# NVIDIA-ISAAC-ROS/isaac_ros_nvblox

Measured on NVIDIA H100. Metric: depth-frames/sec (TSDF+ESDF integrate, 640x480 @ 5 cm voxels), higher is better.
Workload: dtype f32

## Files before the change

### isaac_ros_nvblox_b200/csrc/nvb_esdf_wavex.cu

```cuda
#include "nvb_esdf_wave_common.cuh"

#include <cstdlib>

namespace nvb {

namespace {

#ifndef NVB_WAVEX_THREADS
#define NVB_WAVEX_THREADS 512
#endif
#ifndef NVB_WAVEX_MAXREG
#define NVB_WAVEX_MAXREG 96
#endif
#ifndef NVB_WAVEX_TAIL
#define NVB_WAVEX_TAIL 1
#endif
#ifndef NVB_WAVEX_PROF
#define NVB_WAVEX_PROF 0
#endif
#ifndef NVB_WAVEX_SPEC_HALO
#define NVB_WAVEX_SPEC_HALO 0
#endif
#if NVB_WAVEX_PROF
#define X_PROF_BEGIN() long long tq = clock64();
#define X_PROF(i) \
  if (lane64 == 0) xs.prof[group][i] += clock64() - tq; \
  tq = clock64();
#define X_PROF_COUNT(i) \
  if (lane64 == 0) xs.prof[group][i]++;
#else
#define X_PROF_BEGIN()
#define X_PROF(i)
#define X_PROF_COUNT(i)
#endif
constexpr int kXT = NVB_WAVEX_THREADS;
constexpr int kXG = kXT / 64;
constexpr int kRecInts = 32;
constexpr int kMaxCtas = 192;
constexpr int kRX = 110, kRY = 11;
constexpr int kRegionVox = 1100;
constexpr int kFlagBase = 4 * kRegionVox;
constexpr int kXRegionWords = 5 * kRegionVox;
constexpr size_t kXSmemBytes = (size_t)kXG * kXRegionWords * sizeof(unsigned int);

struct XTables {
  unsigned int halo[8][64];
  unsigned int pair[6][4][64];
};

struct XShared {
  int rec[kXG][kRecInts];
  int nb[kXG][8];
  int pos[kXG][8];
  unsigned int mask[kXG];
  int changed[kXG];
  unsigned int live[kXG][8];
  int seg[kXG][2];
  int pre[kMaxCtas + 1];
  int warp_tot[2][8];
  int ncand, nchanged;
  int next;
  int cur[kXG];
  int seeds[kXG];
  int bcast[4];
  unsigned int generation;
  int n_bar;
  int ring;
  int swept, faces, rings, n_tail;
#if NVB_WAVEX_PROF
  long long prof[kXG][8];
#endif
};

struct XCtx {
  unsigned char* blocks;
  int* block_index;
  DevHash hash;
  int* nbr;
  int* nbr27;
  int* cand_stamp;
  unsigned int* psum;
  int* stamp[2];
  unsigned char* X[2];
  int* recs[2];
  int seg;
  int* error;
  float max_sq;
  __device__ __forceinline__ int* segment(int p, int cta) const { return recs[p] + (size_t)cta * seg * kRecInts; }
};

__shared__ XTables x_tab;
__shared__ XShared x_xs;
__shared__ XCtx x_ctx;
extern __shared__ __align__(16) unsigned int x_smem[];

__device__ __forceinline__ int rvox(int rx, int ry, int rz) { return rx * kRX + ry * kRY + rz; }
__device__ __forceinline__ int faceEntry(int f) {
  return f == 0 ? 22 : (f == 1 ? 4 : (f == 2 ? 16 : (f == 3 ? 10 : (f == 4 ? 14 : 12))));
}
__device__ __forceinline__ int boundaryOff(int r) { return r == 0 ? -1 : (r == 9 ? 1 : 0); }
__device__ __forceinline__ int boundaryLoc(int r) { return r == 0 ? 7 : (r == 9 ? 0 : r - 1); }

__device__ __forceinline__ int neighbor27(const XCtx& c, int slot, int d) {
  int v = __ldcg(c.nbr27 + 27 * slot + d);
  if (v < -1) {
    const int* bi = c.block_index + 3 * slot;
    v = (d == 13) ? slot : hashFind(c.hash, bi[0] + d / 9 - 1, bi[1] + (d / 3) % 3 - 1, bi[2] + d % 3 - 1);
    c.nbr27[27 * slot + d] = v;
  }
  return v;
}
__device__ __forceinline__ int neighbor6(const XCtx& c, int slot, int dir) {
  int v = __ldcg(c.nbr + 6 * slot + dir);
  if (v < -1) {
    const int* bi = c.block_index + 3 * slot;
    const int d = (dir & 1) ? -1 : 1;
    v = hashFind(c.hash, bi[0] + ((dir >> 1) == 0 ? d : 0), bi[1] + ((dir >> 1) == 1 ? d : 0), bi[2] + ((dir >> 1) == 2 ? d : 0));
    c.nbr[6 * slot + dir] = v;
  }
  return v;
}

__device__ __forceinline__ void initTables(XTables& tab, int tid) {
  for (int i = tid; i < 512; i += kXT) {
    const int k = i >> 6, lane = i & 63;
    unsigned int e = 0;
    int ra = 1, r1 = 1, r2 = 1, axis = 0;
    bool valid = true;
    if (k < 6) {
      axis = k >> 1;
      ra = (k & 1) ? 0 : 9, r1 = (lane >> 3) + 1, r2 = (lane & 7) + 1;
    } else {
      const int n = i - 384;
      if (n < 96) {
        const int edge = n >> 3, cn = edge & 3;
        axis = edge >> 2;
        ra = (n & 7) + 1, r1 = (cn & 1) ? 9 : 0, r2 = (cn & 2) ? 9 : 0;
      } else if (n < 104) {
        const int cn = n - 96;
        ra = (cn & 1) ? 9 : 0, r1 = (cn & 2) ? 9 : 0, r2 = (cn & 4) ? 9 : 0;
      } else {
        valid = false;
      }
    }
    if (valid) {
      const int rx = axis == 0 ? ra : r1, ry = axis == 0 ? r1 : (axis == 1 ? ra : r2), rz = axis == 2 ? ra : r2;
      const int d = (boundaryOff(rx) + 1) * 9 + (boundaryOff(ry) + 1) * 3 + (boundaryOff(rz) + 1);
      e = (unsigned)rvox(rx, ry, rz) | ((unsigned)(boundaryLoc(rx) * 64 + boundaryLoc(ry) * 8 + boundaryLoc(rz)) << 11) |
          ((unsigned)d << 20) | (1u << 25);
    }
    tab.halo[k][lane] = e;
  }
  for (int i = tid; i < 6 * 4 * 64; i += kXT) {
    const int pass = i >> 8, j = (i >> 6) & 3, lane = i & 63;
    const int axis = pass >> 1, dir = (pass & 1) ? -1 : 1;
    int plane, u, w;
    bool valid = true;
    if (j < 2) {
      plane = j, u = (lane >> 3) + 1, w = (lane & 7) + 1;
    } else {
      const int n = (j - 2) * 64 + lane;
      plane = n / 36;
      const int q = n % 36;
      if (q < 10) u = 0, w = q;
      else if (q < 20) u = 9, w = q - 10;
      else if (q < 28) u = q - 20 + 1, w = 0;
      else u = q - 28 + 1, w = 9;
      if (n >= 72) valid = false, plane = 0, u = 1, w = 1;
    }
    unsigned int e = 0;
    if (valid) {
      const int sa = dir > 0 ? (plane ? 8 : 0) : (plane ? 9 : 1);
      const int so = dir > 0 ? (plane ? 0 : -1) : (plane ? 1 : 0);
      const int da = sa + dir;
      const int A = axis == 0 ? 9 : (axis == 1 ? 3 : 1), U = axis == 0 ? 3 : 9, W = axis == 2 ? 3 : 1;
      const int d = 13 + so * A + boundaryOff(u) * U + boundaryOff(w) * W;
      const int inner = da >= 1 && da <= 8 && u >= 1 && u <= 8 && w >= 1 && w <= 8;
      const int sv = axis == 0 ? rvox(sa, u, w) : (axis == 1 ? rvox(u, sa, w) : rvox(u, w, sa));
      const int dv = axis == 0 ? rvox(da, u, w) : (axis == 1 ? rvox(u, da, w) : rvox(u, w, da));
      e = (unsigned)sv | ((unsigned)dv << 11) | ((unsigned)d << 22) | ((unsigned)inner << 27) | (1u << 28);
    }
    tab.pair[pass][j][lane] = e;
  }
}

struct LiveMasks {
  unsigned int* live;
  unsigned int needed;
};
__device__ __forceinline__ LiveMasks liveMasks(unsigned int mask, unsigned int* live_smem, bool writer) {
  LiveMasks L;
  L.live = live_smem;
  const unsigned int ok = mask | (1u << 13);
  const unsigned int D[6] = {0x7FFFE00u, 0x3FE00u, 0x3F000u, 0x7000u, 0x6000u, 0x2000u};
  unsigned int acc = 0;
#pragma unroll
  for (int p = 0; p < 6; p++) {
    const int axis = p >> 1;
    const int A = axis == 0 ? 9 : (axis == 1 ? 3 : 1);
    const unsigned int lo = axis == 0 ? 0x000001ffu : (axis == 1 ? 0x001c0e07u : 0x01249249u);
    const unsigned int dst_ok = ok & D[p];
    unsigned int lv, dst;
    if ((p & 1) == 0) {
      lv = mask & (lo | (lo << A)) & (dst_ok >> A);
      dst = lv << A;
    } else {
      lv = mask & ((lo << A) | (lo << (2 * A))) & (dst_ok << A);
      dst = lv >> A;
    }
    if (writer) live_smem[p] = lv;
    acc |= lv | dst;
  }
  L.needed = acc & mask & ~(1u << 13);
  return L;
}

struct OwnRegs {
  uint4 q[10];
};
__device__ __forceinline__ OwnRegs ownLoad(const unsigned char* blk, int lane64) {
  OwnRegs o;
  const uint4* src = reinterpret_cast<const uint4*>(blk) + lane64 * 10;
#pragma unroll
  for (int i = 0; i < 10; i++) o.q[i] = __ldcg(src + i);
  return o;
}
__device__ __forceinline__ unsigned int ownWord(const OwnRegs& o, int w) {
  const uint4& v = o.q[w >> 2];
  return (w & 3) == 0 ? v.x : ((w & 3) == 1 ? v.y : ((w & 3) == 2 ? v.z : v.w));
}
__device__ __forceinline__ void ownToShared(unsigned int* R, const OwnRegs& o, int lane64) {
  uint4* A = reinterpret_cast<uint4*>(R);
  const int v0 = rvox((lane64 >> 3) + 1, (lane64 & 7) + 1, 1);
#pragma unroll
  for (int z = 0; z < 8; z++) {
    A[v0 + z] = make_uint4(ownWord(o, 5 * z), ownWord(o, 5 * z + 1), ownWord(o, 5 * z + 2), ownWord(o, 5 * z + 3));
    R[kFlagBase + v0 + z] = ownWord(o, 5 * z + 4);
  }
}
__device__ __forceinline__ void ownStore(unsigned char* layer_blk, bool to_layer, unsigned char* x_blk, const unsigned int* R,
                                         unsigned int* psum_slot, int lane64) {
  const uint4* A = reinterpret_cast<const uint4*>(R);
  const int x = lane64 >> 3, y = lane64 & 7;
  const int v0 = rvox(x + 1, y + 1, 1);
  uint4* dl = reinterpret_cast<uint4*>(layer_blk) + lane64 * 10;
  uint4* dx = reinterpret_cast<uint4*>(x_blk) + lane64 * 10;
  int lo0 = 99, lo1 = 99, lo2 = 99, hi0 = -99, hi1 = -99, hi2 = -99;
#pragma unroll
  for (int h = 0; h < 2; h++) {
    unsigned int w[20];
#pragma unroll
    for (int z = 0; z < 4; z++) {
      const uint4 a = A[v0 + 4 * h + z];
      w[5 * z] = a.x, w[5 * z + 1] = a.y, w[5 * z + 2] = a.z, w[5 * z + 3] = a.w;
      w[5 * z + 4] = R[kFlagBase + v0 + 4 * h + z];
      if ((a.y | a.z | a.w) != 0u) {
        const int b0 = (x + (int)a.y) >> 3, b1 = (y + (int)a.z) >> 3, b2 = (4 * h + z + (int)a.w) >> 3;
        lo0 = min(lo0, b0), hi0 = max(hi0, b0), lo1 = min(lo1, b1), hi1 = max(hi1, b1), lo2 = min(lo2, b2), hi2 = max(hi2, b2);
      }
    }
#pragma unroll
    for (int i = 0; i < 5; i++) {
      const uint4 v = make_uint4(w[4 * i], w[4 * i + 1], w[4 * i + 2], w[4 * i + 3]);
      if (to_layer) __stcg(dl + 5 * h + i, v);
      __stcg(dx + 5 * h + i, v);
    }
  }
  if (psum_slot) {
    lo0 = __reduce_min_sync(0xffffffffu, lo0), lo1 = __reduce_min_sync(0xffffffffu, lo1), lo2 = __reduce_min_sync(0xffffffffu, lo2);
    hi0 = __reduce_max_sync(0xffffffffu, hi0), hi1 = __reduce_max_sync(0xffffffffu, hi1), hi2 = __reduce_max_sync(0xffffffffu, hi2);
    if ((lane64 & 31) == 0) {
      unsigned int v = 0u;
      if (lo0 <= hi0) {
        const bool fits = lo0 >= -16 && lo1 >= -16 && lo2 >= -16 && hi0 <= 15 && hi1 <= 15 && hi2 <= 15;
        v = fits ? ((1u << 31) | (unsigned)(lo0 + 16) | ((unsigned)(hi0 + 16) << 5) | ((unsigned)(lo1 + 16) << 10) |
                    ((unsigned)(hi1 + 16) << 15) | ((unsigned)(lo2 + 16) << 20) | ((unsigned)(hi2 + 16) << 25))
                 : 0xffffffffu;
      }
      psum_slot[lane64 >> 5] = v;
    }
  }
}

__device__ __forceinline__ void cpAsync4(unsigned int* smem_dst, const unsigned int* gsrc) {
  asm volatile("cp.async.ca.shared.global [%0], [%1], 4;" ::"r"((unsigned int)__cvta_generic_to_shared(smem_dst)), "l"(gsrc)
               : "memory");
}
__device__ __forceinline__ void haloAsync(const XTables& tab, unsigned int* R, const int* row, const unsigned char* X, int lane64,
                                          unsigned int batches, unsigned int blocks) {
#pragma unroll 1
  while (batches) {
    const int k = __ffs(batches) - 1;
    batches &= batches - 1;
    const unsigned int e = tab.halo[k][lane64];
    const int d = (e >> 20) & 31u;
    const int slot = ((e >> 25) & 1u) && ((blocks >> d) & 1u) ? row[d] : -1;
    if (slot >= 0) {
      const unsigned int* src = reinterpret_cast<const unsigned int*>(X + (size_t)slot * kEsdfBlockBytes) + ((e >> 11) & 511u) * kEsdfVoxelWords;
      const int v = e & 2047u;
#pragma unroll
      for (int w = 0; w < 4; w++) cpAsync4(R + 4 * v + w, src + w);
      cpAsync4(R + kFlagBase + v, src + 4);
    }
  }
}
constexpr unsigned int kFaceBlocks = (1u << 22) | (1u << 4) | (1u << 16) | (1u << 10) | (1u << 14) | (1u << 12);
__device__ __forceinline__ unsigned int haloBatches(unsigned int needed) {
  unsigned int bl = ((needed >> 22) & 1u) | (((needed >> 4) & 1u) << 1) | (((needed >> 16) & 1u) << 2) | (((needed >> 10) & 1u) << 3) |
                    (((needed >> 14) & 1u) << 4) | (((needed >> 12) & 1u) << 5);
  if (needed & ~kFaceBlocks) bl |= 0xC0u;
  return bl;
}

__device__ __forceinline__ bool replayX(const XTables& tab, unsigned int* R, const LiveMasks& L, int lane64, int group,
                                        float max_sq) {
  uint4* A = reinterpret_cast<uint4*>(R);
  const unsigned int* live_p = L.live;
  bool changed = false;
#pragma unroll 1
  for (int pass = 0; pass < 6; pass++) {
    const unsigned int live = live_p[pass];
    if (!live) continue;
    const int axis = pass >> 1, dir = (pass & 1) ? -1 : 1;
    const int s0 = axis == 0 ? dir : 0, s1 = axis == 1 ? dir : 0, s2 = axis == 2 ? dir : 0;
#pragma unroll 1
    for (int j = 0; j < 4; j++) {
      unsigned int e = tab.pair[pass][j][lane64];
      if (!((e >> 28) & 1u) || !((live >> ((e >> 22) & 31u)) & 1u)) e = 0;
      if (__any_sync(0xffffffffu, e != 0u)) {
        const int sv = e & 2047u, dv = (e >> 11) & 2047u;
        const uint4 es = A[sv], ns = A[dv];
        const unsigned int ef = R[kFlagBase + sv], nf = R[kFlagBase + dv];
        const bool ok = e != 0u && flagObserved(ef) && flagObserved(nf) && !flagSite(nf) && !(__uint_as_float(es.x) >= max_sq);
        const int d0 = (int)es.y - s0, d1 = (int)es.z - s1, d2 = (int)es.w - s2;
        const float pdist = (float)(d0 * d0 + (d1 * d1 + d2 * d2));
        if (ok && __uint_as_float(ns.x) > pdist) {
          A[dv] = make_uint4(__float_as_uint(pdist), (unsigned)d0, (unsigned)d1, (unsigned)d2);
          changed = changed || ((e >> 27) & 1u);
        }
      }
    }
    groupSync(group);
  }
  return changed;
}

template <int AXIS>
__device__ __forceinline__ bool sweepLineX(unsigned int* R, int a, int b, float max_sq) {
  uint4* A = reinterpret_cast<uint4*>(R);
  const int v0 = AXIS == 0 ? rvox(1, a + 1, b + 1) : (AXIS == 1 ? rvox(a + 1, 1, b + 1) : rvox(a + 1, b + 1, 1));
  constexpr int stride = AXIS == 0 ? kRX : (AXIS == 1 ? kRY : 1);
  constexpr int kNone = 1 << 28, kCap = 1 << 27;
  int T[kVps], pa[kVps], po1[kVps], po2[kVps], pp2[kVps];
  unsigned int tk = 0, dirty = 0;
#pragma unroll
  for (int i = 0; i < kVps; i++) {
    const uint4 q = A[v0 + i * stride];
    const unsigned int fl = R[kFlagBase + v0 + i * stride];
    const float sq = __uint_as_float(q.x);
    const bool o = flagObserved(fl), st = flagSite(fl);
    const int t = min(__float2int_ru(sq), kCap);
    T[i] = (o && !st) ? t : INT_MIN;
    const int qa = (int)(AXIS == 0 ? q.y : (AXIS == 1 ? q.z : q.w));
    const int q1 = (int)(AXIS == 0 ? q.z : q.y);
    const int q2 = (int)(AXIS == 2 ? q.z : q.w);
    pa[i] = st ? 0 : qa, po1[i] = st ? 0 : q1, po2[i] = st ? 0 : q2;
    pp2[i] = po1[i] * po1[i] + po2[i] * po2[i];
    if (o && (st || sq < max_sq)) tk |= 1u << i;
  }
#pragma unroll
  for (int pass = 0; pass < 2; pass++) {
    int la = 0, lo1 = 0, lo2 = 0, lp2 = kNone;
#pragma unroll
    for (int kk = 0; kk < kVps; kk++) {
      const int k = pass ? (kVps - 1 - kk) : kk;
      const int t = la - k;
      const int pd = t * t + lp2;
      const bool improve = T[k] > pd;
      const bool take = ((tk >> k) & 1u) && !improve;
      const int offer_a = pa[k] + k;
      if (improve) {
        T[k] = pd, pa[k] = t, po1[k] = lo1, po2[k] = lo2, pp2[k] = lp2;
        dirty |= 1u << k;
      }
      la = take ? offer_a : la;
      lo1 = take ? po1[k] : lo1;
      lo2 = take ? po2[k] : lo2;
      lp2 = take ? pp2[k] : lp2;
    }
    tk |= dirty;
  }
#pragma unroll
  for (int i = 0; i < kVps; i++) {
    if ((dirty >> i) & 1u) {
      const unsigned int x = (unsigned)(AXIS == 0 ? pa[i] : po1[i]);
      const unsigned int y = (unsigned)(AXIS == 0 ? po1[i] : (AXIS == 1 ? pa[i] : po2[i]));
      const unsigned int z = (unsigned)(AXIS == 2 ? pa[i] : po2[i]);
      A[v0 + i * stride] = make_uint4(__float_as_uint((float)T[i]), x, y, z);
    }
  }
  return dirty != 0;
}
__device__ __forceinline__ bool sweepBlockX(unsigned int* R, int group, int lane64, float max_sq) {
  const int a = lane64 >> 3, b = lane64 & 7;
  bool ch = sweepLineX<0>(R, a, b, max_sq);
  groupSync(group);
  ch |= sweepLineX<1>(R, a, b, max_sq);
  groupSync(group);
  ch |= sweepLineX<2>(R, a, b, max_sq);
  return ch;
}

struct RegState {
  int old;
  int pos;
  int v[3];
};
__device__ __forceinline__ RegState registerBegin(const XCtx& c, XShared& xs, int group, int lane64, int target) {
  RegState s;
  s.old = target, s.pos = -1;
  if (lane64 < 6) {
    const int nb = xs.nb[group][lane64];
    if (nb >= 0) s.old = atomicExch(c.cand_stamp + nb, target);
  }
#pragma unroll
  for (int k = 0; k < 3; k++) {
    const int idx = lane64 + 64 * k;
    s.v[k] = -1;
    if (idx < 162) {
      const int nb = xs.nb[group][idx / 27];
      if (nb >= 0) s.v[k] = __ldcg(c.nbr27 + 27 * nb + idx % 27);
    }
  }
  return s;
}
__device__ __forceinline__ void registerClaim(const XCtx& c, XShared& xs, RegState& s, int group, int lane64, int target) {
  if (lane64 < 32) {
    const bool win = lane64 < 6 && xs.nb[group][lane64] >= 0 && s.old != target;
    const unsigned int ballot = __ballot_sync(0xffffffffu, win);
    if (ballot) {
      int base = 0;
      if (lane64 == 0) base = atomicAdd(&xs.ncand, __popc(ballot));
      base = __shfl_sync(0xffffffffu, base, 0);
      if (win) s.pos = base + __popc(ballot & ((1u << lane64) - 1u));
      if (s.pos >= c.seg) {
        s.pos = -1;
        atomicOr(c.error, 8);
      }
    }
  }
}
__device__ __forceinline__ void registerFinish(const XCtx& c, XShared& xs, const RegState& s, int group, int lane64,
                                               int* segment) {
  if (lane64 < 6) xs.pos[group][lane64] = s.pos;
  groupSync(group);
#pragma unroll
  for (int k = 0; k < 3; k++) {
    const int idx = lane64 + 64 * k;
    if (idx < 162) {
      const int w = idx / 27, pos = xs.pos[group][w];
      if (pos >= 0) {
        int v = s.v[k];
        if (v < -1) v = neighbor27(c, xs.nb[group][w], idx % 27);
        __stcg(segment + (size_t)pos * kRecInts + 1 + idx % 27, v);
      }
    }
  }
  if (lane64 < 6 && s.pos >= 0) __stcg(segment + (size_t)s.pos * kRecInts, xs.nb[group][lane64]);
}

__device__ __noinline__ void processCandidate(int ring) {
  const XCtx& c = x_ctx;
  const XTables& tab = x_tab;
  XShared& xs = x_xs;
  const int cta = blockIdx.x, group = threadIdx.x >> 6, lane64 = threadIdx.x & 63;
  unsigned int* R = x_smem + group * kXRegionWords;
  const int ci = ring & 1, ni = ci ^ 1;
  X_PROF_BEGIN()
  if (lane64 < 28) xs.rec[group][lane64] = __ldcg(c.segment(ci, xs.seg[group][0]) + (size_t)xs.seg[group][1] * kRecInts + lane64);
  groupSync(group);
  X_PROF(0)
  const int slot = xs.rec[group][0];
  const int* row = &xs.rec[group][1];
  int sv = ring - 1;
  if (lane64 < 27 && row[lane64] >= 0) sv = __ldcg(c.stamp[ci] + row[lane64]);
  OwnRegs own = ownLoad(c.blocks + (size_t)slot * kEsdfBlockBytes, lane64);
  if (NVB_WAVEX_SPEC_HALO) haloAsync(tab, R, row, c.X[ci], lane64, 0x3Fu, 0x7FFFFFFu);
  const unsigned int m = __ballot_sync(0xffffffffu, lane64 < 27 && sv == ring);
  if (lane64 == 0) xs.mask[group] = m, xs.changed[group] = 0;
  ownToShared(R, own, lane64);
  if (NVB_WAVEX_SPEC_HALO) cpAsyncWaitAll();
  groupSync(group);
  const LiveMasks L = liveMasks(xs.mask[group], xs.live[group], lane64 == 0);
  X_PROF(1)
  const unsigned int rest = NVB_WAVEX_SPEC_HALO ? (L.needed & ~kFaceBlocks) : L.needed;
  if (rest) {
    haloAsync(tab, R, row, c.X[ci], lane64, haloBatches(rest), rest);
    cpAsyncWaitAll();
  }
  groupSync(group);
  X_PROF(2)
  const bool ch = replayX(tab, R, L, lane64, group, c.max_sq);
  if (ch) xs.changed[group] = 1;
  groupSync(group);
  X_PROF(3)
  X_PROF_COUNT(6)
  if (xs.changed[group]) {
    if (lane64 < 6) xs.nb[group][lane64] = row[faceEntry(lane64)];
    if (lane64 == 0) {
      __stcg(c.stamp[ni] + slot, ring + 1);
      atomicAdd(&xs.nchanged, 1);
    }
    groupSync(group);
    RegState rs = registerBegin(c, xs, group, lane64, ring + 1);
    sweepBlockX(R, group, lane64, c.max_sq);
    registerClaim(c, xs, rs, group, lane64, ring + 1);
    groupSync(group);
    X_PROF(4)
    ownStore(c.blocks + (size_t)slot * kEsdfBlockBytes, true, c.X[ni] + (size_t)slot * kEsdfBlockBytes, R, c.psum + 2 * (size_t)slot, lane64);
    registerFinish(c, xs, rs, group, lane64, c.segment(ni, cta));
    X_PROF_COUNT(7)
  }
  groupSync(group);
  X_PROF(5)
}

__device__ __noinline__ void processSeed(int ring, int slot) {
  const XCtx& c = x_ctx;
  XShared& xs = x_xs;
  const int cta = blockIdx.x, group = threadIdx.x >> 6, lane64 = threadIdx.x & 63;
  unsigned int* R = x_smem + group * kXRegionWords;
  const int ci = ring & 1;
  unsigned char* blk = c.blocks + (size_t)slot * kEsdfBlockBytes;
  OwnRegs own = ownLoad(blk, lane64);
  if (lane64 < 6) xs.nb[group][lane64] = neighbor6(c, slot, lane64);
  if (lane64 == 0) {
    __stcg(c.stamp[ci] + slot, ring);
    xs.changed[group] = 0;
  }
  groupSync(group);
  RegState rs = registerBegin(c, xs, group, lane64, ring);
  ownToShared(R, own, lane64);
  groupSync(group);
  const bool ch = sweepBlockX(R, group, lane64, c.max_sq);
  registerClaim(c, xs, rs, group, lane64, ring);
  if (ch) xs.changed[group] = 1;
  groupSync(group);
  ownStore(blk, xs.changed[group] != 0, c.X[ci] + (size_t)slot * kEsdfBlockBytes, R, xs.changed[group] ? c.psum + 2 * (size_t)slot : nullptr, lane64);
  registerFinish(c, xs, rs, group, lane64, c.segment(ci, cta));
  groupSync(group);
}

#ifndef NVB_WAVEX_BARRIER_RA
#define NVB_WAVEX_BARRIER_RA 1
#endif
__device__ __forceinline__ void gridBarrierRA(unsigned int* bar, unsigned int& generation, unsigned int nctas) {
  __syncthreads();
  if (threadIdx.x == 0) {
    generation++;
    const unsigned int target = generation * nctas;
    asm volatile("red.release.gpu.global.add.u32 [%0], 1;" ::"l"(bar) : "memory");
    unsigned int v;
    do {
      asm volatile("ld.acquire.gpu.global.u32 %0, [%1];" : "=r"(v) : "l"(bar) : "memory");
    } while (v < target);
  }
  __syncthreads();
}

__device__ __forceinline__ void counterBarrierScan(XShared& xs, unsigned int* bar, unsigned int& generation, int2* counts, int nctas,
                                                   int cta, int tid, int seg, int ring_inc, int* K, int* M) {
  counts += (xs.n_bar & 1) * kMaxCtas;
  __syncthreads();
  if (tid == 0) {
    __stcg(counts + cta, make_int2(min(xs.ncand, seg), xs.nchanged));
    xs.ncand = 0, xs.nchanged = 0;
  }
  if (NVB_WAVEX_BARRIER_RA)
    gridBarrierRA(bar, generation, nctas);
  else
    gridBarrier(bar, generation, nctas);
  int2 v = make_int2(0, 0);
  if (tid < nctas) v = __ldcg(counts + tid);
  const int lane = tid & 31, warp = tid >> 5;
  int inc = v.x, chg = v.y;
#pragma unroll
  for (int o = 1; o < 32; o <<= 1) {
    const int t = __shfl_up_sync(0xffffffffu, inc, o);
    if (lane >= o) inc += t;
  }
#pragma unroll
  for (int o = 16; o > 0; o >>= 1) chg += __shfl_xor_sync(0xffffffffu, chg, o);
  if (warp < 8 && lane == 31) xs.warp_tot[0][warp] = inc;
  if (warp < 8 && lane == 0) xs.warp_tot[1][warp] = chg;
  __syncthreads();
  int base = 0, mtot = 0;
#pragma unroll
  for (int w = 0; w < 8; w++) {
    if (w < warp) base += xs.warp_tot[0][w];
    if (w * 32 < nctas) mtot += xs.warp_tot[1][w];
  }
  if (tid < nctas) xs.pre[tid + 1] = base + inc;
  if (tid == 0) xs.pre[0] = 0, xs.next = 0, xs.ring += ring_inc, xs.n_bar++;
  __syncthreads();
  *K = xs.pre[nctas];
  *M = mtot;
}

__global__ void __maxnreg__(NVB_WAVEX_MAXREG) esdfWaveXKernel(EsdfCtx c) {
  XShared& xs = x_xs;
  const int cta = blockIdx.x, nctas = gridDim.x;
  const int tid = threadIdx.x, group = tid >> 6, lane64 = tid & 63;
  if (*(volatile int*)c.work_count == 0) return;
  initTables(x_tab, tid);
  if (tid == 0) {
    xs.ncand = 0, xs.nchanged = 0, xs.next = 0;
    xs.ring = *(volatile int*)c.ring_id;
    xs.generation = 0, xs.n_bar = 0, xs.swept = 0, xs.faces = 0, xs.rings = 0, xs.n_tail = 0;
    XCtx& xc = x_ctx;
    xc.blocks = c.esdf.blocks, xc.block_index = c.esdf.block_index, xc.hash = c.esdf.hash;
    xc.nbr = c.nbr, xc.nbr27 = c.nbr27, xc.cand_stamp = c.cand_stamp, xc.psum = c.psum;
    xc.stamp[0] = c.stamp_a, xc.stamp[1] = c.stamp_b;
    xc.X[0] = c.xslab, xc.X[1] = c.xslab + (size_t)c.esdf.capacity * kEsdfBlockBytes;
    xc.recs[0] = c.xrec, xc.recs[1] = c.xrec + (size_t)nctas * c.xseg * kRecInts;
    xc.seg = c.xseg, xc.error = c.error, xc.max_sq = c.max_sq;
  }
#if NVB_WAVEX_PROF
  if (lane64 < 8) xs.prof[group][lane64] = 0;
#endif
  __syncthreads();
#if NVB_WAVEX_PROF
  long long t_bar = 0, t_work = 0, t0 = globalTimerNs(), t1;
  int dbgK = 0, dbgM = 0;
#define X_DBG(k, m) dbgK = (k), dbgM = (m);
#define X_TIME_WORK()                                                                                                      \
  t1 = globalTimerNs(), t_work += t1 - t0;                                                                                 \
  if (tid == 0 && xs.n_bar < 1000) atomicMax((unsigned long long*)c.phase_max + xs.n_bar, (unsigned long long)(t1 - t0)); \
  if (cta == 0 && tid == 0 && xs.n_bar < 1000)                                                                             \
    c.phase_max[1000 + xs.n_bar] = dbgK, c.phase_max[2000 + xs.n_bar] = dbgM, c.phase_max[3000 + xs.n_bar] = t1 - t0;      \
  t0 = t1;
#define X_TIME_BARRIER() t1 = globalTimerNs(), t_bar += t1 - t0, t0 = t1;
#else
#define X_DBG(k, m)
#define X_TIME_WORK()
#define X_TIME_BARRIER()
#endif
#define X_BARRIER(inc, Kout, Mout)                                                                                        \
  X_TIME_WORK()                                                                                                           \
  counterBarrierScan(xs, c.barrier, xs.generation, reinterpret_cast<int2*>(c.xcounts), nctas, cta, tid, c.xseg, inc,        \
                     &(Kout), &(Mout));                                                                                   \
  X_TIME_BARRIER()
  for (int pass = 0; pass < 2; pass++) {
    const int* src = pass ? c.cleared_list : c.upd_list;
    const int n0 = pass ? *(volatile int*)c.cleared_count : *(volatile int*)c.upd_count;
    if (n0 == 0) continue;
    X_DBG(-1, n0)
    if (lane64 == 0) xs.seeds[group] = n0;
    for (;;) {
      if (lane64 == 0) xs.cur[group] = atomicAdd(&xs.next, 1);
      groupSync(group);
      const long long e = (long long)cta + (long long)xs.cur[group] * nctas;
      if (e >= xs.seeds[group]) break;
      processSeed(xs.ring, __ldcg(src + e));
    }
    int M = xs.seeds[group], K, unused;
    X_BARRIER(0, K, unused)
    if (tid == 0) xs.swept += M;
    while (true) {
      X_DBG(K, M)
      if (NVB_WAVEX_TAIL && K <= kXG) {
        if (cta == 0) {
          int t = 0;
          if (group < K) {
            for (int s = lane64; s < nctas; s += 64)
              if (xs.pre[s] <= group && group < xs.pre[s + 1]) xs.seg[group][0] = s, xs.seg[group][1] = group - xs.pre[s];
          }
          __syncthreads();
          while (true) {
            if (group < K) processCandidate(xs.ring);
            __syncthreads();
            const int K2 = min(xs.ncand, c.xseg), M2 = xs.nchanged;
            __syncthreads();
            if (tid == 0) xs.ncand = 0, xs.nchanged = 0, xs.faces += 6 * M, xs.rings++, xs.swept += M2, xs.ring++;
            if (tid < kXG) xs.seg[tid][0] = 0, xs.seg[tid][1] = tid;
            t++;
            M = M2, K = K2;
            __syncthreads();
            if (M == 0 || K > kXG) break;
          }
          if (tid == 0) xs.n_tail += t, c.xtail[0] = t, c.xtail[1] = K, c.xtail[2] = M;
        }
        {
          int k_unused, m_unused;
          X_BARRIER(0, k_unused, m_unused)
        }
        if (cta != 0) {
          if (tid == 0) xs.bcast[0] = __ldcg(c.xtail + 0), xs.bcast[1] = __ldcg(c.xtail + 1), xs.bcast[2] = __ldcg(c.xtail + 2);
          __syncthreads();
          K = xs.bcast[1], M = xs.bcast[2];
          if (tid == 0) xs.ring += xs.bcast[0];
          __syncthreads();
        }
        if (M == 0) break;
        for (int s = tid; s <= nctas; s += kXT) xs.pre[s] = s == 0 ? 0 : K;
        __syncthreads();
        continue;
      }
      for (;;) {
        if (lane64 == 0) xs.cur[group] = atomicAdd(&xs.next, 1);
        groupSync(group);
        const long long e = (long long)cta + (long long)xs.cur[group] * nctas;
        if (e >= K) break;
        for (int s = lane64; s < nctas; s += 64)
          if (xs.pre[s] <= e && e < xs.pre[s + 1]) xs.seg[group][0] = s, xs.seg[group][1] = (int)e - xs.pre[s];
        groupSync(group);
        processCandidate(xs.ring);
      }
      int K2, M2;
      X_BARRIER(1, K2, M2)
      if (tid == 0) xs.faces += 6 * M, xs.rings++, xs.swept += M2;
      M = M2, K = K2;
      if (M == 0) break;
    }
    if (tid == 0) xs.ring++;
    __syncthreads();
  }
#undef X_BARRIER
#undef X_TIME_WORK
#undef X_TIME_BARRIER
#undef X_DBG
  if (cta == 0 && tid == 0) {
    *c.ring_id = xs.ring + 1;
    c.stats[4] = *(volatile int*)c.cleared_count;
    c.stats[5] = xs.swept, c.stats[6] = xs.faces, c.stats[7] = xs.rings;
    c.stats[10] = xs.n_tail, c.stats[11] = xs.n_bar;
#if NVB_WAVEX_PROF
    c.stats[8] = t_bar, c.stats[9] = t_work;
    long long sum_max = 0;
    for (int q = 0; q < xs.n_bar && q < 1000; q++) sum_max += (long long)c.phase_max[q];
    c.stats[12] = sum_max;
    for (int q = 0; q < 8; q++) c.phase_max[3990 + q] = xs.prof[0][q];
#endif
  }
}

}

int esdfWaveXGrid(int num_sms, int reserved_sms) {
  int grid = num_sms < kMaxCtas ? num_sms : kMaxCtas;
  if (reserved_sms > 0 && grid - reserved_sms >= 8) grid -= reserved_sms;
  return grid;
}
size_t esdfWaveXFlagBytes() { return 2 * (size_t)kMaxCtas * sizeof(int2); }

cudaError_t launchEsdfComputeX(const EsdfCtx& c, int num_sms, int reserved_sms, cudaStream_t stream, int* launches) {
  static int per_sm = -1;
  if (per_sm < 0) {
    cudaFuncSetAttribute(esdfWaveXKernel, cudaFuncAttributeMaxDynamicSharedMemorySize, (int)kXSmemBytes);
    int v = 0;
    if (cudaOccupancyMaxActiveBlocksPerMultiprocessor(&v, esdfWaveXKernel, kXT, kXSmemBytes) != cudaSuccess) v = 0;
    per_sm = v;
  }
  if (per_sm <= 0) return cudaErrorLaunchOutOfResources;
  EsdfCtx cc = c;
  void* args[] = {&cc};
  (*launches)++;
  const int grid = esdfWaveXGrid(num_sms, reserved_sms);
  return cudaLaunchCooperativeKernel((const void*)esdfWaveXKernel, dim3(grid), dim3(kXT), args, kXSmemBytes, stream);
}

}
```

Baseline: 2693.

## Coalesce own-block loads, remap shared scatter, and L2-prefetch neighbor blocks

```diff
diff --git a/isaac_ros_nvblox_b200/csrc/nvb_esdf_wavex.cu b/isaac_ros_nvblox_b200/csrc/nvb_esdf_wavex.cu
--- a/isaac_ros_nvblox_b200/csrc/nvb_esdf_wavex.cu
+++ b/isaac_ros_nvblox_b200/csrc/nvb_esdf_wavex.cu
@@ -17,9 +17,6 @@
 #endif
 #ifndef NVB_WAVEX_PROF
 #define NVB_WAVEX_PROF 0
-#endif
-#ifndef NVB_WAVEX_SPEC_HALO
-#define NVB_WAVEX_SPEC_HALO 0
 #endif
 #if NVB_WAVEX_PROF
 #define X_PROF_BEGIN() long long tq = clock64();
@@ -220,22 +217,33 @@
 };
 __device__ __forceinline__ OwnRegs ownLoad(const unsigned char* blk, int lane64) {
   OwnRegs o;
-  const uint4* src = reinterpret_cast<const uint4*>(blk) + lane64 * 10;
-#pragma unroll
-  for (int i = 0; i < 10; i++) o.q[i] = __ldcg(src + i);
+  const uint4* src = reinterpret_cast<const uint4*>(blk) + lane64;
+#pragma unroll
+  for (int i = 0; i < 10; i++) o.q[i] = __ldcg(src + 64 * i);
   return o;
 }
 __device__ __forceinline__ unsigned int ownWord(const OwnRegs& o, int w) {
   const uint4& v = o.q[w >> 2];
   return (w & 3) == 0 ? v.x : ((w & 3) == 1 ? v.y : ((w & 3) == 2 ? v.z : v.w));
 }
+__device__ __forceinline__ int rvoxOf(unsigned int v) { return (int)(v + 3u * (v >> 3) + 22u * (v >> 6)) + kRX + kRY + 1; }
 __device__ __forceinline__ void ownToShared(unsigned int* R, const OwnRegs& o, int lane64) {
-  uint4* A = reinterpret_cast<uint4*>(R);
-  const int v0 = rvox((lane64 >> 3) + 1, (lane64 & 7) + 1, 1);
-#pragma unroll
-  for (int z = 0; z < 8; z++) {
-    A[v0 + z] = make_uint4(ownWord(o, 5 * z), ownWord(o, 5 * z + 1), ownWord(o, 5 * z + 2), ownWord(o, 5 * z + 3));
-    R[kFlagBase + v0 + z] = ownWord(o, 5 * z + 4);
+#pragma unroll
+  for (int i = 0; i < 5; i++) {
+    unsigned int l;
+    asm("min.u32 %0, %1, %2;" : "=r"(l) : "r"((unsigned int)lane64), "r"(o.q[i].w | 64u));
+    const unsigned int w0 = 256u * i + 4u * l, v0 = (w0 * 52429u) >> 18, f0 = w0 - 5u * v0;
+    const int r0 = rvoxOf(v0), r1 = rvoxOf(v0 + 1u);
+#pragma unroll
+    for (int j = 0; j < 4; j++) {
+      const unsigned int f = f0 + j;
+      const bool next = f >= 5u;
+      const int r = next ? r1 : r0;
+      const unsigned int g = next ? f - 5u : f;
+      const int a = g < 4u ? 4 * r + (int)g : kFlagBase + r;
+      R[a] = ownWord(o, 4 * i + j);
+      R[a + (g < 4u ? 4 * 4 * kRX : 4 * kRX)] = ownWord(o, 4 * (i + 5) + j);
+    }
   }
 }
 __device__ __forceinline__ void ownStore(unsigned char* layer_blk, bool to_layer, unsigned char* x_blk, const unsigned int* R,
@@ -411,6 +419,10 @@
   return ch;
 }
 
+__device__ __forceinline__ void prefetchL2(const void* gsrc, unsigned int bytes) {
+  asm volatile("cp.async.bulk.prefetch.L2.global [%0], %1;" ::"l"(gsrc), "r"(bytes) : "memory");
+}
+
 struct RegState {
   int old;
   int pos;
@@ -421,7 +433,10 @@
   s.old = target, s.pos = -1;
   if (lane64 < 6) {
     const int nb = xs.nb[group][lane64];
-    if (nb >= 0) s.old = atomicExch(c.cand_stamp + nb, target);
+    if (nb >= 0) {
+      prefetchL2(c.blocks + (size_t)nb * kEsdfBlockBytes, kEsdfBlockBytes);
+      s.old = atomicExch(c.cand_stamp + nb, target);
+    }
   }
 #pragma unroll
   for (int k = 0; k < 3; k++) {
@@ -485,17 +500,14 @@
   int sv = ring - 1;
   if (lane64 < 27 && row[lane64] >= 0) sv = __ldcg(c.stamp[ci] + row[lane64]);
   OwnRegs own = ownLoad(c.blocks + (size_t)slot * kEsdfBlockBytes, lane64);
-  if (NVB_WAVEX_SPEC_HALO) haloAsync(tab, R, row, c.X[ci], lane64, 0x3Fu, 0x7FFFFFFu);
   const unsigned int m = __ballot_sync(0xffffffffu, lane64 < 27 && sv == ring);
   if (lane64 == 0) xs.mask[group] = m, xs.changed[group] = 0;
   ownToShared(R, own, lane64);
-  if (NVB_WAVEX_SPEC_HALO) cpAsyncWaitAll();
   groupSync(group);
   const LiveMasks L = liveMasks(xs.mask[group], xs.live[group], lane64 == 0);
   X_PROF(1)
-  const unsigned int rest = NVB_WAVEX_SPEC_HALO ? (L.needed & ~kFaceBlocks) : L.needed;
-  if (rest) {
-    haloAsync(tab, R, row, c.X[ci], lane64, haloBatches(rest), rest);
+  if (L.needed) {
+    haloAsync(tab, R, row, c.X[ci], lane64, haloBatches(L.needed), L.needed);
     cpAsyncWaitAll();
   }
   groupSync(group);
```

Measured after the change: 2727, median of 6. 1.2% higher.
